# ymLuo1214/RAFT-Stereo

Measured on AMD Instinct MI355X. Metric: stereo pairs/s at 540x960, 32 iters, 1-8 GPUs; corr-lookup HBM GB/s, higher is better.
Workload: dtype f32; 1 GPU; corr path: CorrBlock1D build + 32 lookups, 540x960 -> 135x240 fmaps, batch 8/GPU, fp32, 4 levels, radius 4; config=sceneflow, global_batch=8, W2=240, levels=4, radius=4, iters=32, parallelism=batch-shard x1, corr_out_layout=nchw, pyramid_layout=rows, coords_field=random

## Files before the change

raft-stereo_amd/csrc/lookup_pair.h:

```cpp
#pragma once
#include <type_traits>

#include "common.h"
#include "lookup_level.h"

namespace rc {

template <class OT>
__device__ __forceinline__ OT out_cvt(float v) {
    if constexpr (std::is_same<OT, float>::value) {
        return v;
    } else {
        asm("" : "+v"(v));
        return (OT)v;
    }
}

template <int S>
__device__ __forceinline__ float pool_tree(const float *v) {
    if constexpr (S == 1) return v[0];
    else return (pool_tree<S / 2>(v) + pool_tree<S / 2>(v + S / 2)) * 0.5f;
}

template <int SI>
__device__ __forceinline__ float derived_elem(const float *row1, long long k) {
    float v[SI];
#pragma unroll
    for (int c = 0; c < SI; ++c) v[c] = row1[SI * k + c];
    return pool_tree<SI>(v);
}

template <int R, bool BF16 = false>
struct PairSpan {
    static constexpr int NW = 2 * R + 4;
    static constexpr int NS = 2 * NW;
    static constexpr int EPC = BF16 ? 8 : 4;
    static constexpr int ES = BF16 ? 2 : 4;
    static constexpr int NC = (NS + EPC - 2 + EPC - 1) / EPC;
    uint32_t q[NC][4];
    float m, n;
    int sh;
    bool inwin, valid;
    __device__ __forceinline__ float elem(int e) const {
        if constexpr (BF16) {
            const uint32_t u = q[e >> 3][(e & 7) >> 1];
            return __builtin_bit_cast(float, (e & 1) ? (u & 0xFFFF0000u) : (u << 16));
        } else {
            return __builtin_bit_cast(float, q[e >> 2][e & 3]);
        }
    }
};

template <int R>
__device__ __forceinline__ void tap_span(float xl, int W, int &f, int &l) {
    const float Wm1 = (float)(W - 1), half = Wm1 / 2.0f;
    const DivRN dv = div_prep(Wm1);
    const float pa = ((div_rn(2.0f * ((float)(-R) + xl), dv) - 1.0f) + 1.0f) * half;
    const float pb = ((div_rn(2.0f * ((float)R + xl), dv) - 1.0f) + 1.0f) * half;
    f = max((int)floorf(pa), 0);
    l = min((int)floorf(pb) + 1, W - 1);
}

template <int R, bool BF16 = false>
__device__ __forceinline__ void issue_pair(PairSpan<R, BF16> &ps, const LookupArgs &a, int lo, float x,
                                           long long pblk, long long lrow) {
    typedef PairSpan<R, BF16> PS;
    const int Wlo = a.W[lo], Whi = a.W[lo + 1];
    const float xlo = x / (float)(1 << lo), xhi = x / (float)(2 << lo);
    ps.inwin = (xhi > -(float)(R + 4)) && (xhi < (float)(Whi + R + 4));
    ps.m = ps.inwin ? floorf(xhi) : 0.0f;
    ps.n = ps.inwin ? floorf(xlo) : 0.0f;
    const int dd = (int)ps.n - 2 * (int)ps.m;
    ps.valid = ps.inwin && (dd == 0 || dd == 1);
    int lo_e = 0x7FFFFFFF, hi_e = -1;
    if (ps.inwin) {
        int f, l;
        tap_span<R>(xlo, Wlo, f, l);
        if (f <= l) { lo_e = f; hi_e = l; }
        tap_span<R>(xhi, Whi, f, l);
        if (f <= l) { lo_e = min(lo_e, 2 * f); hi_e = max(hi_e, 2 * l + 1); }
    }
    const int sa = 2 * ((int)ps.m - R - 1);
    const int ea = sa & ~(PS::EPC - 1);
    ps.sh = sa - ea;
    const long long ld = a.ld[lo];
    const char *lvl = static_cast<const char *>(a.lvl[lo]);
    const long long shb = a.shadow[lo];
    const auto rs = make_rsrc(lvl + pblk * ld * PS::ES, clamp_bytes((a.P - pblk) * ld * PS::ES + shb));
    uint32_t phase = 0;
    if (shb != 0 && lo_e <= hi_e) {
        const unsigned long long b0 =
            (unsigned long long)(uintptr_t)(lvl + ((pblk + lrow) * ld + (lo_e & ~(PS::EPC - 1))) * PS::ES);
        const unsigned long long b1 = (unsigned long long)(uintptr_t)(lvl + ((pblk + lrow) * ld + hi_e) * PS::ES);
        const unsigned long long sh = (unsigned long long)shb;
        const long long l0 = (long long)(b1 >> 7) - (long long)(b0 >> 7);
        const long long l1 = (long long)((b1 + sh) >> 7) - (long long)((b0 + sh) >> 7);
        phase = l1 < l0 ? (uint32_t)sh : 0u;
    }
#pragma unroll
    for (int k = 0; k < PS::NC; ++k) {
        const int cs = ea + PS::EPC * k;
        const bool ok = cs <= hi_e && cs + PS::EPC - 1 >= lo_e;
        const auto v = __builtin_amdgcn_raw_buffer_load_b128(
            rs, ok ? (int)((uint32_t)((lrow * ld + cs) * PS::ES) + phase) : (int)0xFFFFFF00u, 0, 0);
#pragma unroll
        for (int c = 0; c < 4; ++c) ps.q[k][c] = v[c];
    }
}

template <int R>
__device__ __forceinline__ void window_taps(const float *w, float xl, float nwin, int W,
                                            float *res) {
    constexpr int T = 2 * R + 1;
    const float Wm1 = (float)(W - 1), half = Wm1 / 2.0f;
    const DivRN dv = div_prep(Wm1);
#pragma unroll
    for (int t = 0; t < T; ++t) {
        const float xt = (float)(t - R) + xl;
        const float xn = div_rn(2.0f * xt, dv) - 1.0f;
        const float xp = (xn + 1.0f) * half;
        const float x0 = floorf(xp);
        const float w1 = xp - x0, w0 = 1.0f - w1;
        const float nt = nwin + (float)(t - R);
        const bool lo_ = x0 < nt, hi_ = x0 > nt;
        float e0 = w[t], e1 = w[t + 1], e2 = w[t + 2], e3 = w[t + 3];
        asm("" : "+v"(e0), "+v"(e1), "+v"(e2), "+v"(e3));
        const float v0 = lo_ ? e0 : (hi_ ? e2 : e1);
        const float v1 = lo_ ? e1 : (hi_ ? e3 : e2);
        res[t] = fmaf(w1, v1, w0 * v0);
    }
}

template <int S>
__device__ __forceinline__ float derived_elem_bf16(const uint16_t *row, long long k) {
    if constexpr (S == 1) {
        return bf16_to_f32(row[k]);
    } else {
        const float a = derived_elem_bf16<S / 2>(row, 2 * k), b = derived_elem_bf16<S / 2>(row, 2 * k + 1);
        return round_bf16((a + b) * 0.5f);
    }
}

template <int R, int S, bool BF16 = false>
__device__ __forceinline__ void level_taps_mem(const void *rowv, float xl, int W, float *res) {
    constexpr int T = 2 * R + 1;
    const float Wm1 = (float)(W - 1), half = Wm1 / 2.0f;
    const DivRN dv = div_prep(Wm1);
    for (int t = 0; t < T; ++t) {
        const float xt = (float)(t - R) + xl;
        const float xn = div_rn(2.0f * xt, dv) - 1.0f;
        const float xp = (xn + 1.0f) * half;
        const float x0 = floorf(xp);
        const float w1 = xp - x0, w0 = 1.0f - w1;
        const bool ok0 = (x0 >= 0.0f) && (x0 <= Wm1);
        const bool ok1 = (x0 + 1.0f >= 0.0f) && (x0 + 1.0f <= Wm1);
        float v0 = 0.0f, v1 = 0.0f;
        if constexpr (BF16) {
            const uint16_t *row = static_cast<const uint16_t *>(rowv);
            if (ok0) v0 = derived_elem_bf16<S>(row, (long long)x0);
            if (ok1) v1 = derived_elem_bf16<S>(row, (long long)x0 + 1);
        } else {
            const float *row = static_cast<const float *>(rowv);
            if (ok0) v0 = derived_elem<S>(row, (long long)x0);
            if (ok1) v1 = derived_elem<S>(row, (long long)x0 + 1);
        }
        res[t] = fmaf(w1, v1, w0 * v0);
    }
}

template <int R, bool NOFALLBACK = false, bool BF16 = false, class Sink>
__device__ __forceinline__ void finish_pair(const PairSpan<R, BF16> &ps, const LookupArgs &a, int lo,
                                            float x, long long pp, Sink &&sink) {
    typedef PairSpan<R, BF16> PS;
    constexpr int T = 2 * R + 1, NW = PS::NW, NS = PS::NS, EPC = PS::EPC;
    const int Wlo = a.W[lo], Whi = a.W[lo + 1];
    float s[NS];
#pragma unroll
    for (int j = 0; j < NS; ++j) {
        float v = ps.elem(j);
#pragma unroll
        for (int d = 2; d < EPC; d += 2)
            if (j + d < PS::NC * EPC) v = (ps.sh == d) ? ps.elem(j + d) : v;
        s[j] = v;
    }
    const int mi = (int)ps.m - R - 1, ni = (int)ps.n - R - 1;
    const int dd = (int)ps.n - 2 * (int)ps.m;
    float wodd[NW], weven[NW];
#pragma unroll
    for (int jj = 0; jj < NW; ++jj) {
        float pm = (s[2 * jj] + s[2 * jj + 1]) * 0.5f;
        if constexpr (BF16) pm = round_bf16(pm);
        wodd[jj] = (unsigned)(mi + jj) < (unsigned)Whi ? pm : 0.0f;
        const float e = dd == 0 ? s[R + 1 + jj] : s[R + 2 + jj];
        weven[jj] = (unsigned)(ni + jj) < (unsigned)Wlo ? e : 0.0f;
    }
    const float xlo = x / (float)(1 << lo), xhi = x / (float)(2 << lo);
    float r0[T], r1[T];
    window_taps<R>(weven, xlo, ps.n, Wlo, r0);
    window_taps<R>(wodd, xhi, ps.m, Whi, r1);
    if (!NOFALLBACK && __builtin_expect(ps.inwin && !ps.valid, 0)) {
        const char *row = static_cast<const char *>(a.lvl[lo]) + pp * a.ld[lo] * PS::ES;
        level_taps_mem<R, 1, BF16>(row, xlo, Wlo, r0);
        level_taps_mem<R, 2, BF16>(row, xhi, Whi, r1);
    }
#pragma unroll
    for (int t = 0; t < T; ++t) sink(lo * T + t, r0[t]);
#pragma unroll
    for (int t = 0; t < T; ++t) sink((lo + 1) * T + t, r1[t]);
}

struct PairPixel {
    long long pblk, pp, lrow;
    long long ooff;
    float x;
    bool active;
};

template <int R, int NL>
__device__ __forceinline__ PairPixel pair_pixel(const LookupArgs &a, long long pblk) {
    PairPixel q;
    q.pblk = pblk;
    const long long p = pblk + threadIdx.x;
    q.active = p < a.P;
    q.pp = q.active ? p : a.P - 1;
    const long long bimg = q.pp / a.HW, rem = q.pp - bimg * a.HW;
    q.x = pixel_x(a, bimg, rem, q.active);
    q.ooff = bimg * (long long)(NL * (2 * R + 1)) * a.HW + rem;
    q.lrow = q.pp - pblk;
    return q;
}

template <int R, int NL, int M = 0, bool BF16 = false, int WPE = 1, bool CL = false, class OT = float>
__global__ __launch_bounds__(256) __attribute__((amdgpu_waves_per_eu(WPE))) void lookup_pair_kernel(LookupArgs a) {
    static_assert(NL == 2 || NL == 4, "pair lookup: 2 or 4 levels");
    constexpr int NP = NL / 2;
    const int blk = M == 5 ? (int)blockIdx.x : xcd_remap(blockIdx.x, gridDim.x);
    const PairPixel q = pair_pixel<R, NL>(a, (long long)blk * 256);
    OT *const outp = reinterpret_cast<OT *>(a.out) + q.ooff;
    PairSpan<R, BF16> sp[NP];
#pragma unroll
    for (int k = 0; k < NP; ++k)
        issue_pair<R, BF16>(sp[k], a, 2 * k, q.x, q.pblk, q.lrow);
    constexpr int C = NL * (2 * R + 1);
    constexpr bool TILE = CL || M == 9;
    __shared__ __attribute__((aligned(16))) OT ctile[TILE ? 4 * 64 * C : 1];
    auto sink = [&](int ch, float v) {
        if constexpr (TILE) {
            ctile[(threadIdx.x >> 6) * 64 * C + (threadIdx.x & 63) * C + ch] = out_cvt<OT>(v);
        } else if constexpr (M == 7) {
            if (q.active) __builtin_nontemporal_store(v, outp + (long long)ch * a.HW);
        } else {
            if (q.active && (M != 1 || v == 1234.5f)) outp[(long long)ch * a.HW] = out_cvt<OT>(v);
        }
    };
#pragma unroll
    for (int k = 0; k < NP; ++k) finish_pair<R, M == 2, BF16>(sp[k], a, 2 * k, q.x, q.pp, sink);
    if constexpr (TILE) {
        constexpr int EPV = 16 / (int)sizeof(OT);
        typedef OT ovec __attribute__((ext_vector_type(EPV)));
        const int lane = threadIdx.x & 63;
        const long long pw = q.pblk + (threadIdx.x & ~63);
        const OT *t = ctile + (threadIdx.x >> 6) * 64 * C;
        OT *const outb = reinterpret_cast<OT *>(a.out);
        const long long lim = (a.P - pw < 64 ? a.P - pw : 64) * C;
#pragma unroll
        for (int k = 0; k < (64 * C / EPV + 63) / 64; ++k) {
            const int e = (k * 64 + lane) * EPV;
            if (e >= 64 * C || e >= lim) continue;
            const ovec v = *reinterpret_cast<const ovec *>(t + e);
            if (e + EPV <= lim) {
                *reinterpret_cast<ovec *>(outb + pw * C + e) = v;
            } else {
#pragma unroll
                for (int j = 0; j < EPV; ++j)
                    if (e + j < lim) outb[pw * C + e + j] = v[j];
            }
        }
    }
}

template <int R, class Sink>
__device__ __forceinline__ void sheared_taps_mem(const LookupArgs &a, int lo, float x, long long bh, int w1,
                                                 Sink &&sink) {
    constexpr int T = 2 * R + 1;
    const float *S = static_cast<const float *>(a.lvl[lo]) + bh * a.shk[lo] * a.ld[lo];
    const int W0 = a.W[lo];
    const long long base = (long long)((w1 >> lo) + W0 - 1);
    auto elem = [&](long long j) { return S[(base - j) * a.ld[lo] + w1]; };
#pragma unroll
    for (int half = 0; half < 2; ++half) {
        const int W = a.W[lo + half];
        const float Wm1 = (float)(W - 1), hw = Wm1 / 2.0f;
        const DivRN dv = div_prep(Wm1);
        const float xl = x / (float)(1 << (lo + half));
        for (int t = 0; t < T; ++t) {
            const float xt = (float)(t - R) + xl;
            const float xn = div_rn(2.0f * xt, dv) - 1.0f;
            const float xp = (xn + 1.0f) * hw;
            const float x0 = floorf(xp);
            const float wt1 = xp - x0, wt0 = 1.0f - wt1;
            const bool ok0 = (x0 >= 0.0f) && (x0 <= Wm1);
            const bool ok1 = (x0 + 1.0f >= 0.0f) && (x0 + 1.0f <= Wm1);
            const long long e = (long long)x0;
            float v0 = 0.0f, v1 = 0.0f;
            if (half == 0) {
                if (ok0) v0 = elem(e);
                if (ok1) v1 = elem(e + 1);
            } else {
                if (ok0) v0 = (elem(2 * e) + elem(2 * e + 1)) * 0.5f;
                if (ok1) v1 = (elem(2 * e + 2) + elem(2 * e + 3)) * 0.5f;
            }
            sink((lo + half) * T + t, fmaf(wt1, v1, wt0 * v0));
        }
    }
}

template <int R, int NL>
__global__ __launch_bounds__(256) void lookup_sheared_pair_kernel(LookupArgs a) {
    static_assert(NL == 2 || NL == 4, "pair lookup: 2 or 4 levels");
    constexpr int NP = NL / 2, NS = PairSpan<R>::NS;
    const int blk = xcd_remap(blockIdx.x, gridDim.x);
    const long long pblk = (long long)blk * 256;
    const long long p = pblk + threadIdx.x;
    const bool active = p < a.P;
    const long long pp = active ? p : a.P - 1;
    const long long bimg = pp / a.HW, rem = pp - bimg * a.HW;
    const float x = pixel_x(a, bimg, rem, active);
    const int H = a.HW / a.W1;
    const int h = (int)(rem / a.W1), w1 = (int)(rem - (long long)h * a.W1);
    const long long bh = bimg * H + h, bh0 = pblk / a.W1;
    float *outp = a.out + bimg * (long long)(NL * (2 * R + 1)) * a.HW + rem;
    auto sink = [&](int ch, float v) {
        if (active) outp[(long long)ch * a.HW] = v;
    };
    PairSpan<R> sp[NP];
#pragma unroll
    for (int k = 0; k < NP; ++k) {
        const int lo = 2 * k;
        PairSpan<R> &ps = sp[k];
        const int Wlo = a.W[lo], Whi = a.W[lo + 1];
        const float xlo = x / (float)(1 << lo), xhi = x / (float)(2 << lo);
        ps.inwin = (xhi > -(float)(R + 4)) && (xhi < (float)(Whi + R + 4));
        ps.m = ps.inwin ? floorf(xhi) : 0.0f;
        ps.n = ps.inwin ? floorf(xlo) : 0.0f;
        const int dd = (int)ps.n - 2 * (int)ps.m;
        ps.valid = ps.inwin && (dd == 0 || dd == 1);
        int lo_e = 0x7FFFFFFF, hi_e = -1;
        if (ps.inwin) {
            int f, l;
            tap_span<R>(xlo, Wlo, f, l);
            if (f <= l) { lo_e = f; hi_e = l; }
            tap_span<R>(xhi, Whi, f, l);
            if (f <= l) { lo_e = min(lo_e, 2 * f); hi_e = max(hi_e, 2 * l + 1); }
        }
        ps.sh = 0;
        const int sa = 2 * ((int)ps.m - R - 1);
        const long long K = a.shk[lo], ldw = a.ld[lo];
        const float *lv = static_cast<const float *>(a.lvl[lo]);
        const auto rs = make_rsrc(lv + bh0 * K * ldw, clamp_bytes((a.P / a.W1 - bh0) * K * ldw * 4));
        const long long rowk = (bh - bh0) * K + (w1 >> lo) + Wlo - 1;
#pragma unroll
        for (int c = 0; c < PairSpan<R>::NC * 4; ++c) {
            const int j = sa + c;
            const bool ok = c < NS && j >= lo_e && j <= hi_e;
            const uint32_t off = ok ? (uint32_t)(((rowk - j) * ldw + w1) * 4) : 0xFFFFFF00u;
            ps.q[c >> 2][c & 3] = __builtin_amdgcn_raw_buffer_load_b32(rs, (int)off, 0, 0);
        }
    }
#pragma unroll
    for (int k = 0; k < NP; ++k) {
        if (__builtin_expect(sp[k].inwin && !sp[k].valid, 0)) {
            sheared_taps_mem<R>(a, 2 * k, x, bh, w1, sink);
            continue;
        }
        finish_pair<R, true>(sp[k], a, 2 * k, x, pp, sink);
    }
}


template <int R>
__device__ __forceinline__ int plan_record_pair(PairSpan<R, true> &ps, const LookupArgs &a, int lo, float x,
                                                int e_first, int slot_first, uint32_t &okmask) {
    typedef PairSpan<R, true> PS;
    const int Wlo = a.W[lo], Whi = a.W[lo + 1];
    const float xlo = x / (float)(1 << lo), xhi = x / (float)(2 << lo);
    ps.inwin = (xhi > -(float)(R + 4)) && (xhi < (float)(Whi + R + 4));
    ps.m = ps.inwin ? floorf(xhi) : 0.0f;
    ps.n = ps.inwin ? floorf(xlo) : 0.0f;
    const int dd = (int)ps.n - 2 * (int)ps.m;
    ps.valid = ps.inwin && (dd == 0 || dd == 1);
    int lo_e = 0x7FFFFFFF, hi_e = -1;
    if (ps.inwin) {
        int f, l;
        tap_span<R>(xlo, Wlo, f, l);
        if (f <= l) { lo_e = f; hi_e = l; }
        tap_span<R>(xhi, Whi, f, l);
        if (f <= l) { lo_e = min(lo_e, 2 * f); hi_e = max(hi_e, 2 * l + 1); }
    }
    const int sslot = 2 * ((int)ps.m - R - 1) - e_first + slot_first;
    const int cb = sslot >= 0 ? sslot & ~7 : -((-sslot + 7) & ~7);
    ps.sh = sslot - cb;
    const int slo = lo_e - e_first + slot_first, shi = hi_e - e_first + slot_first;
    okmask = 0;
#pragma unroll
    for (int k = 0; k < PS::NC; ++k) {
        const int cs = cb + 8 * k;
        if (lo_e <= hi_e && cs <= shi && cs + 7 >= slo && cs >= 0 && cs + 8 <= kRecSlots) okmask |= 1u << k;
    }
    return cb;
}

template <int R, bool NOLOAD = false>
__device__ __forceinline__ void issue_record_pair(PairSpan<R, true> &ps, const LookupArgs &a, int lo, float x,
                                                  const __amdgpu_buffer_rsrc_t &rs, uint32_t rbyte, int e_first,
                                                  int slot_first) {
    typedef PairSpan<R, true> PS;
    uint32_t okm;
    const int cb = plan_record_pair<R>(ps, a, lo, x, e_first, slot_first, okm);
#pragma unroll
    for (int k = 0; k < PS::NC; ++k) {
        const int cs = cb + 8 * k;
        const bool ok = (okm >> k) & 1u;
        if constexpr (NOLOAD) {
            uint32_t o = ok ? rbyte + 2u * (uint32_t)cs : 0u;
            asm volatile("" : "+v"(o));
#pragma unroll
            for (int c = 0; c < 4; ++c) ps.q[k][c] = o + c;
        } else {
            const auto v = __builtin_amdgcn_raw_buffer_load_b128(
                rs, ok ? (int)(rbyte + 2u * (uint32_t)cs) : (int)0xFFFFFF00u, 0, 0);
#pragma unroll
            for (int c = 0; c < 4; ++c) ps.q[k][c] = v[c];
        }
    }
}

template <int R>
__device__ __forceinline__ void lds_record_pair(PairSpan<R, true> &ps, const LookupArgs &a, int lo, float x,
                                                const char *rec, int e_first, int slot_first) {
    typedef PairSpan<R, true> PS;
    uint32_t okm;
    const int cb = plan_record_pair<R>(ps, a, lo, x, e_first, slot_first, okm);
#pragma unroll
    for (int k = 0; k < PS::NC; ++k) {
        const int cs = cb + 8 * k;
        uint4 v = uint4{0u, 0u, 0u, 0u};
        if ((okm >> k) & 1u) v = *reinterpret_cast<const uint4 *>(rec + 2 * cs);
        ps.q[k][0] = v.x;
        ps.q[k][1] = v.y;
        ps.q[k][2] = v.z;
        ps.q[k][3] = v.w;
    }
}

template <int R, class Sink>
__device__ __forceinline__ void record_taps_mem(const LookupArgs &a, const uint16_t *rec, int lo, float x,
                                                Sink &&sink) {
    constexpr int T = 2 * R + 1;
    const int NR = a.rec_nr;
    auto elem = [&](long long e) {
        int r = lo == 0 ? (int)((e - rec_e0(0)) >> 4) : (int)((e - rec_e2(0)) >> 2);
        r = r < NR ? r : NR - 1;
        const int slot = lo == 0 ? kRecL2Slots + (int)e - rec_e0(r) : (int)e - rec_e2(r);
        return bf16_to_f32(rec[r * kRecSlots + slot]);
    };
#pragma unroll
    for (int half = 0; half < 2; ++half) {
        const int W = a.W[lo + half];
        const float Wm1 = (float)(W - 1), hw = Wm1 / 2.0f;
        const DivRN dv = div_prep(Wm1);
        const float xl = x / (float)(1 << (lo + half));
        for (int t = 0; t < T; ++t) {
            const float xt = (float)(t - R) + xl;
            const float xn = div_rn(2.0f * xt, dv) - 1.0f;
            const float xp = (xn + 1.0f) * hw;
            const float x0 = floorf(xp);
            const float wt1 = xp - x0, wt0 = 1.0f - wt1;
            const bool ok0 = (x0 >= 0.0f) && (x0 <= Wm1);
            const bool ok1 = (x0 + 1.0f >= 0.0f) && (x0 + 1.0f <= Wm1);
            const long long e = (long long)x0;
            float v0 = 0.0f, v1 = 0.0f;
            if (half == 0) {
                if (ok0) v0 = elem(e);
                if (ok1) v1 = elem(e + 1);
            } else {
                if (ok0) v0 = round_bf16((elem(2 * e) + elem(2 * e + 1)) * 0.5f);
                if (ok1) v1 = round_bf16((elem(2 * e + 2) + elem(2 * e + 3)) * 0.5f);
            }
            sink((lo + half) * T + t, fmaf(wt1, v1, wt0 * v0));
        }
    }
}

template <int R, bool CL, int M = 0, bool COOP = false, int WPE = 1, class OT = float>
__global__ __launch_bounds__(256) __attribute__((amdgpu_waves_per_eu(WPE))) void lookup_records_kernel(LookupArgs a) {
    constexpr int NL = 4, C = NL * (2 * R + 1);
    const int blk = xcd_remap(blockIdx.x, gridDim.x);
    const PairPixel q = pair_pixel<R, NL>(a, (long long)blk * 256);
    const int NR = a.rec_nr;
    float mf = floorf(q.x / 2.0f);
    mf = fminf(fmaxf(mf, (float)kRecM0), (float)(kRecM0 + 8 * NR - 1));
    const int r = ((int)mf - kRecM0) >> 3;
    const uint16_t *blkrec = static_cast<const uint16_t *>(a.lvl[0]) + q.pblk * (long long)NR * kRecSlots;
    const auto rs = make_rsrc(blkrec, clamp_bytes((a.P - q.pblk) * (long long)NR * kRecSlots * 2));
    const uint32_t rbyte = (uint32_t)((q.lrow * NR + r) * kRecSlots * 2);
    PairSpan<R, true> sp[2];
    constexpr int TB = 64 * C * (int)sizeof(OT);
    constexpr int WB = CL ? (COOP && TB < 8192 ? 8192 : TB) : (COOP ? 8192 : 16);
    __shared__ __attribute__((aligned(16))) char lds[4 * WB];
    char *wlds = lds + (threadIdx.x >> 6) * WB;
    if constexpr (COOP) {
        typedef __attribute__((address_space(3))) void lds_void;
        const int lane = threadIdx.x & 63;
#pragma unroll
        for (int k = 0; k < 8; ++k) {
            const uint32_t rb = (uint32_t)__shfl((int)rbyte, 8 * k + (lane >> 3), 64);
            const int wp = (int)(threadIdx.x & ~63) + 8 * k + (lane >> 3);
            const uint32_t off = q.pblk + wp < a.P ? rb + 16u * (uint32_t)(lane & 7) : 0xFFFFFF00u;
            __builtin_amdgcn_raw_ptr_buffer_load_lds(rs, (lds_void *)(wlds + 1024 * k), 16, (int)off, 0, 0, 0);
        }
        asm volatile("s_waitcnt vmcnt(0)" ::: "memory");
        const char *myrec = wlds + 128 * lane;
        lds_record_pair<R>(sp[0], a, 0, q.x, myrec, rec_e0(r), kRecL2Slots);
        lds_record_pair<R>(sp[1], a, 2, q.x, myrec, rec_e2(r), 0);
        asm volatile("s_waitcnt lgkmcnt(0)" ::: "memory");
    } else {
        issue_record_pair<R, M == 2>(sp[0], a, 0, q.x, rs, rbyte, rec_e0(r), kRecL2Slots);
        issue_record_pair<R, M == 2>(sp[1], a, 2, q.x, rs, rbyte, rec_e2(r), 0);
    }
    if constexpr (M == 3) {
        uint32_t acc = 0;
#pragma unroll
        for (int k = 0; k < 2; ++k)
#pragma unroll
            for (int j = 0; j < PairSpan<R, true>::NC; ++j) acc ^= sp[k].q[j][0] ^ sp[k].q[j][1] ^ sp[k].q[j][2] ^ sp[k].q[j][3];
        asm volatile("" ::"v"(acc));
        return;
    }
    OT *const ctw = reinterpret_cast<OT *>(wlds);
    OT *const outp = reinterpret_cast<OT *>(a.out) + q.ooff;
    auto sink = [&](int ch, float v) {
        if constexpr (CL) ctw[(threadIdx.x & 63) * C + ch] = out_cvt<OT>(v);
        else if (q.active) outp[(long long)ch * a.HW] = out_cvt<OT>(v);
    };
#pragma unroll
    for (int k = 0; k < 2; ++k) {
        if (__builtin_expect(sp[k].inwin && !sp[k].valid, 0)) {
            record_taps_mem<R>(a, blkrec + q.lrow * (long long)NR * kRecSlots, 2 * k, q.x, sink);
            continue;
        }
        finish_pair<R, true, true>(sp[k], a, 2 * k, q.x, q.pp, sink);
    }
    if constexpr (CL) {
        const int lane = threadIdx.x & 63;
        const long long pw = q.pblk + (threadIdx.x & ~63);
        constexpr int EPV = 16 / (int)sizeof(OT);
        typedef OT ovec __attribute__((ext_vector_type(EPV)));
        const OT *t = ctw;
        OT *const outb = reinterpret_cast<OT *>(a.out);
        const long long lim = (a.P - pw < 64 ? a.P - pw : 64) * C;
#pragma unroll
        for (int k = 0; k < (64 * C / EPV + 63) / 64; ++k) {
            const int e = (k * 64 + lane) * EPV;
            if (e >= 64 * C || e >= lim) continue;
            const ovec v = *reinterpret_cast<const ovec *>(t + e);
            if constexpr (M == 1) {
                asm volatile("" ::"v"(v));
            } else if (e + EPV <= lim) {
                *reinterpret_cast<ovec *>(outb + pw * C + e) = v;
            } else {
#pragma unroll
                for (int j = 0; j < EPV; ++j)
                    if (e + j < lim) outb[pw * C + e + j] = v[j];
            }
        }
    }
}

}
```

Baseline: 8405 pairs/s.

## Stagger second level-pair loads behind first pair's tap compute and reuse endpoint taps

The pair kernel now plans and issues the buffer loads for the first level pair, then defers the second pair's loads until after the first pair's even-level taps have been emitted. Scheduling barriers pin this order so the second pair's memory latency can overlap compute while fewer registers are live at once. Tap-span endpoint positions are computed once in a shared planning helper and reused for the first and last taps in window_taps, which removes duplicated divisions. The changes add scheduling constraints that could serialise work if the compiler's own ordering was already better.

```diff
diff --git a/raft-stereo_amd/csrc/lookup_pair.h b/raft-stereo_amd/csrc/lookup_pair.h
--- a/raft-stereo_amd/csrc/lookup_pair.h
+++ b/raft-stereo_amd/csrc/lookup_pair.h
@@ -39,6 +39,7 @@
     static constexpr int NC = (NS + EPC - 2 + EPC - 1) / EPC;
     uint32_t q[NC][4];
     float m, n;
+    float xe[4];
     int sh;
     bool inwin, valid;
     __device__ __forceinline__ float elem(int e) const {
@@ -51,20 +52,24 @@
     }
 };
 
-template <int R>
-__device__ __forceinline__ void tap_span(float xl, int W, int &f, int &l) {
-    const float Wm1 = (float)(W - 1), half = Wm1 / 2.0f;
-    const DivRN dv = div_prep(Wm1);
-    const float pa = ((div_rn(2.0f * ((float)(-R) + xl), dv) - 1.0f) + 1.0f) * half;
-    const float pb = ((div_rn(2.0f * ((float)R + xl), dv) - 1.0f) + 1.0f) * half;
-    f = max((int)floorf(pa), 0);
-    l = min((int)floorf(pb) + 1, W - 1);
-}
-
-template <int R, bool BF16 = false>
-__device__ __forceinline__ void issue_pair(PairSpan<R, BF16> &ps, const LookupArgs &a, int lo, float x,
-                                           long long pblk, long long lrow) {
-    typedef PairSpan<R, BF16> PS;
+struct LevelConsts {
+    float Wm1, half;
+    DivRN dv;
+};
+__device__ __forceinline__ LevelConsts level_consts(const LookupArgs &a, int i) {
+    const float Wm1 = (float)(a.W[i] - 1);
+    return LevelConsts{Wm1, Wm1 / 2.0f, div_prep(Wm1)};
+}
+
+__device__ __forceinline__ float tap_xp(float xl, int k, const LevelConsts &c) {
+    const float xt = (float)k + xl;
+    const float xn = div_rn(2.0f * xt, c.dv) - 1.0f;
+    return (xn + 1.0f) * c.half;
+}
+
+template <int R, bool BF16>
+__device__ __forceinline__ void plan_pair(PairSpan<R, BF16> &ps, const LookupArgs &a, int lo, float x,
+                                          int &lo_e, int &hi_e) {
     const int Wlo = a.W[lo], Whi = a.W[lo + 1];
     const float xlo = x / (float)(1 << lo), xhi = x / (float)(2 << lo);
     ps.inwin = (xhi > -(float)(R + 4)) && (xhi < (float)(Whi + R + 4));
@@ -72,21 +77,42 @@
     ps.n = ps.inwin ? floorf(xlo) : 0.0f;
     const int dd = (int)ps.n - 2 * (int)ps.m;
     ps.valid = ps.inwin && (dd == 0 || dd == 1);
-    int lo_e = 0x7FFFFFFF, hi_e = -1;
+    const LevelConsts clo = level_consts(a, lo), chi = level_consts(a, lo + 1);
+    ps.xe[0] = tap_xp(xlo, -R, clo);
+    ps.xe[1] = tap_xp(xlo, R, clo);
+    ps.xe[2] = tap_xp(xhi, -R, chi);
+    ps.xe[3] = tap_xp(xhi, R, chi);
+    lo_e = 0x7FFFFFFF;
+    hi_e = -1;
     if (ps.inwin) {
-        int f, l;
-        tap_span<R>(xlo, Wlo, f, l);
+        int f = max((int)floorf(ps.xe[0]), 0), l = min((int)floorf(ps.xe[1]) + 1, Wlo - 1);
         if (f <= l) { lo_e = f; hi_e = l; }
-        tap_span<R>(xhi, Whi, f, l);
+        f = max((int)floorf(ps.xe[2]), 0);
+        l = min((int)floorf(ps.xe[3]) + 1, Whi - 1);
         if (f <= l) { lo_e = min(lo_e, 2 * f); hi_e = max(hi_e, 2 * l + 1); }
     }
+}
+
+template <int R, bool BF16>
+struct PairLoads {
+    __amdgpu_buffer_rsrc_t rs;
+    int off[PairSpan<R, BF16>::NC];
+};
+
+template <int R, bool BF16 = false>
+__device__ __forceinline__ PairLoads<R, BF16> plan_pair_loads(PairSpan<R, BF16> &ps, const LookupArgs &a, int lo,
+                                                              float x, long long pblk, long long lrow) {
+    typedef PairSpan<R, BF16> PS;
+    int lo_e, hi_e;
+    plan_pair<R, BF16>(ps, a, lo, x, lo_e, hi_e);
     const int sa = 2 * ((int)ps.m - R - 1);
     const int ea = sa & ~(PS::EPC - 1);
     ps.sh = sa - ea;
     const long long ld = a.ld[lo];
     const char *lvl = static_cast<const char *>(a.lvl[lo]);
     const long long shb = a.shadow[lo];
-    const auto rs = make_rsrc(lvl + pblk * ld * PS::ES, clamp_bytes((a.P - pblk) * ld * PS::ES + shb));
+    PairLoads<R, BF16> pl;
+    pl.rs = make_rsrc(lvl + pblk * ld * PS::ES, clamp_bytes((a.P - pblk) * ld * PS::ES + shb));
     uint32_t phase = 0;
     if (shb != 0 && lo_e <= hi_e) {
         const unsigned long long b0 =
@@ -101,32 +127,40 @@
     for (int k = 0; k < PS::NC; ++k) {
         const int cs = ea + PS::EPC * k;
         const bool ok = cs <= hi_e && cs + PS::EPC - 1 >= lo_e;
-        const auto v = __builtin_amdgcn_raw_buffer_load_b128(
-            rs, ok ? (int)((uint32_t)((lrow * ld + cs) * PS::ES) + phase) : (int)0xFFFFFF00u, 0, 0);
+        pl.off[k] = ok ? (int)((uint32_t)((lrow * ld + cs) * PS::ES) + phase) : (int)0xFFFFFF00u;
+    }
+    return pl;
+}
+
+template <int R, bool BF16>
+__device__ __forceinline__ void load_pair(PairSpan<R, BF16> &ps, const PairLoads<R, BF16> &pl) {
+#pragma unroll
+    for (int k = 0; k < PairSpan<R, BF16>::NC; ++k) {
+        const auto v = __builtin_amdgcn_raw_buffer_load_b128(pl.rs, pl.off[k], 0, 0);
 #pragma unroll
         for (int c = 0; c < 4; ++c) ps.q[k][c] = v[c];
     }
 }
 
 template <int R>
-__device__ __forceinline__ void window_taps(const float *w, float xl, float nwin, int W,
-                                            float *res) {
-    constexpr int T = 2 * R + 1;
-    const float Wm1 = (float)(W - 1), half = Wm1 / 2.0f;
-    const DivRN dv = div_prep(Wm1);
+__device__ __forceinline__ void window_taps(const float *w, float xl, float nwin, const LevelConsts &lc,
+                                            float xa, float xb, float *res) {
+    constexpr int T = 2 * R + 1, NW = 2 * R + 4;
+    float e[NW];
+#pragma unroll
+    for (int j = 0; j < NW; ++j) {
+        e[j] = w[j];
+        asm("" : "+v"(e[j]));
+    }
 #pragma unroll
     for (int t = 0; t < T; ++t) {
-        const float xt = (float)(t - R) + xl;
-        const float xn = div_rn(2.0f * xt, dv) - 1.0f;
-        const float xp = (xn + 1.0f) * half;
+        const float xp = t == 0 ? xa : (t == T - 1 ? xb : tap_xp(xl, t - R, lc));
         const float x0 = floorf(xp);
         const float w1 = xp - x0, w0 = 1.0f - w1;
         const float nt = nwin + (float)(t - R);
         const bool lo_ = x0 < nt, hi_ = x0 > nt;
-        float e0 = w[t], e1 = w[t + 1], e2 = w[t + 2], e3 = w[t + 3];
-        asm("" : "+v"(e0), "+v"(e1), "+v"(e2), "+v"(e3));
-        const float v0 = lo_ ? e0 : (hi_ ? e2 : e1);
-        const float v1 = lo_ ? e1 : (hi_ ? e3 : e2);
+        const float v0 = lo_ ? e[t] : (hi_ ? e[t + 2] : e[t + 1]);
+        const float v1 = lo_ ? e[t + 1] : (hi_ ? e[t + 3] : e[t + 2]);
         res[t] = fmaf(w1, v1, w0 * v0);
     }
 }
@@ -142,14 +176,11 @@
 }
 
 template <int R, int S, bool BF16 = false>
-__device__ __forceinline__ void level_taps_mem(const void *rowv, float xl, int W, float *res) {
+__device__ __forceinline__ void level_taps_mem(const void *rowv, float xl, const LevelConsts &lc, float *res) {
     constexpr int T = 2 * R + 1;
-    const float Wm1 = (float)(W - 1), half = Wm1 / 2.0f;
-    const DivRN dv = div_prep(Wm1);
+    const float Wm1 = lc.Wm1;
     for (int t = 0; t < T; ++t) {
-        const float xt = (float)(t - R) + xl;
-        const float xn = div_rn(2.0f * xt, dv) - 1.0f;
-        const float xp = (xn + 1.0f) * half;
+        const float xp = tap_xp(xl, t - R, lc);
         const float x0 = floorf(xp);
         const float w1 = xp - x0, w0 = 1.0f - w1;
         const bool ok0 = (x0 >= 0.0f) && (x0 <= Wm1);
@@ -168,24 +199,31 @@
     }
 }
 
-template <int R, bool NOFALLBACK = false, bool BF16 = false, class Sink>
-__device__ __forceinline__ void finish_pair(const PairSpan<R, BF16> &ps, const LookupArgs &a, int lo,
-                                            float x, long long pp, Sink &&sink) {
+template <int R, bool BF16>
+__device__ __forceinline__ void span_shift(const PairSpan<R, BF16> &ps, float *s) {
     typedef PairSpan<R, BF16> PS;
-    constexpr int T = 2 * R + 1, NW = PS::NW, NS = PS::NS, EPC = PS::EPC;
+#pragma unroll
+    for (int j = 0; j < PS::NS; ++j) {
+        float v = ps.elem(j);
+#pragma unroll
+        for (int d = 2; d < PS::EPC; d += 2)
+            if (j + d < PS::NC * PS::EPC) v = (ps.sh == d) ? ps.elem(j + d) : v;
+        s[j] = v;
+    }
+}
+
+template <int R, bool NOFALLBACK = false, bool BF16 = false, class Sink, class Mid>
+__device__ __forceinline__ void finish_span(const PairSpan<R, BF16> &ps, const float *s, const LookupArgs &a,
+                                            int lo, float x, long long pp, Sink &&sink, Mid &&mid) {
+    typedef PairSpan<R, BF16> PS;
+    constexpr int T = 2 * R + 1, NW = PS::NW;
     const int Wlo = a.W[lo], Whi = a.W[lo + 1];
-    float s[NS];
-#pragma unroll
-    for (int j = 0; j < NS; ++j) {
-        float v = ps.elem(j);
-#pragma unroll
-        for (int d = 2; d < EPC; d += 2)
-            if (j + d < PS::NC * EPC) v = (ps.sh == d) ? ps.elem(j + d) : v;
-        s[j] = v;
-    }
     const int mi = (int)ps.m - R - 1, ni = (int)ps.n - R - 1;
     const int dd = (int)ps.n - 2 * (int)ps.m;
-    float wodd[NW], weven[NW];
+    const float xlo = x / (float)(1 << lo), xhi = x / (float)(2 << lo);
+    const bool mem = !NOFALLBACK && ps.inwin && !ps.valid;
+    const char *row = static_cast<const char *>(a.lvl[lo]) + pp * a.ld[lo] * PS::ES;
+    float weven[NW], wodd[NW];
 #pragma unroll
     for (int jj = 0; jj < NW; ++jj) {
         float pm = (s[2 * jj] + s[2 * jj + 1]) * 0.5f;
@@ -194,19 +232,25 @@
         const float e = dd == 0 ? s[R + 1 + jj] : s[R + 2 + jj];
         weven[jj] = (unsigned)(ni + jj) < (unsigned)Wlo ? e : 0.0f;
     }
-    const float xlo = x / (float)(1 << lo), xhi = x / (float)(2 << lo);
-    float r0[T], r1[T];
-    window_taps<R>(weven, xlo, ps.n, Wlo, r0);
-    window_taps<R>(wodd, xhi, ps.m, Whi, r1);
-    if (!NOFALLBACK && __builtin_expect(ps.inwin && !ps.valid, 0)) {
-        const char *row = static_cast<const char *>(a.lvl[lo]) + pp * a.ld[lo] * PS::ES;
-        level_taps_mem<R, 1, BF16>(row, xlo, Wlo, r0);
-        level_taps_mem<R, 2, BF16>(row, xhi, Whi, r1);
-    }
-#pragma unroll
-    for (int t = 0; t < T; ++t) sink(lo * T + t, r0[t]);
-#pragma unroll
-    for (int t = 0; t < T; ++t) sink((lo + 1) * T + t, r1[t]);
+    const LevelConsts clo = level_consts(a, lo), chi = level_consts(a, lo + 1);
+    float r[T];
+    window_taps<R>(weven, xlo, ps.n, clo, ps.xe[0], ps.xe[1], r);
+    if (__builtin_expect(mem, 0)) level_taps_mem<R, 1, BF16>(row, xlo, clo, r);
+#pragma unroll
+    for (int t = 0; t < T; ++t) sink(lo * T + t, r[t]);
+    mid();
+    window_taps<R>(wodd, xhi, ps.m, chi, ps.xe[2], ps.xe[3], r);
+    if (__builtin_expect(mem, 0)) level_taps_mem<R, 2, BF16>(row, xhi, chi, r);
+#pragma unroll
+    for (int t = 0; t < T; ++t) sink((lo + 1) * T + t, r[t]);
+}
+
+template <int R, bool NOFALLBACK = false, bool BF16 = false, class Sink>
+__device__ __forceinline__ void finish_pair(const PairSpan<R, BF16> &ps, const LookupArgs &a, int lo,
+                                            float x, long long pp, Sink &&sink) {
+    float s[PairSpan<R, BF16>::NS];
+    span_shift<R, BF16>(ps, s);
+    finish_span<R, NOFALLBACK, BF16>(ps, s, a, lo, x, pp, sink, [] {});
 }
 
 struct PairPixel {
@@ -238,9 +282,11 @@
     const PairPixel q = pair_pixel<R, NL>(a, (long long)blk * 256);
     OT *const outp = reinterpret_cast<OT *>(a.out) + q.ooff;
     PairSpan<R, BF16> sp[NP];
-#pragma unroll
-    for (int k = 0; k < NP; ++k)
-        issue_pair<R, BF16>(sp[k], a, 2 * k, q.x, q.pblk, q.lrow);
+    PairLoads<R, BF16> pl[NP];
+    pl[0] = plan_pair_loads<R, BF16>(sp[0], a, 0, q.x, q.pblk, q.lrow);
+    load_pair<R, BF16>(sp[0], pl[0]);
+    __builtin_amdgcn_sched_barrier(0);
+    if constexpr (NP > 1) pl[1] = plan_pair_loads<R, BF16>(sp[1], a, 2, q.x, q.pblk, q.lrow);
     constexpr int C = NL * (2 * R + 1);
     constexpr bool TILE = CL || M == 9;
     __shared__ __attribute__((aligned(16))) OT ctile[TILE ? 4 * 64 * C : 1];
@@ -254,7 +300,21 @@
         }
     };
 #pragma unroll
-    for (int k = 0; k < NP; ++k) finish_pair<R, M == 2, BF16>(sp[k], a, 2 * k, q.x, q.pp, sink);
+    for (int k = 0; k < NP; ++k) {
+        float s[PairSpan<R, BF16>::NS];
+        span_shift<R, BF16>(sp[k], s);
+        auto next = [&] {
+            if constexpr (NP > 1) {
+                if (k == 0) {
+                    __builtin_amdgcn_sched_barrier(0);
+                    load_pair<R, BF16>(sp[1], pl[1]);
+                    __builtin_amdgcn_sched_barrier(0);
+                }
+            }
+        };
+        finish_span<R, M == 2, BF16>(sp[k], s, a, 2 * k, q.x, q.pp, sink, next);
+        __builtin_amdgcn_sched_barrier(0);
+    }
     if constexpr (TILE) {
         constexpr int EPV = 16 / (int)sizeof(OT);
         typedef OT ovec __attribute__((ext_vector_type(EPV)));
@@ -289,14 +349,11 @@
     auto elem = [&](long long j) { return S[(base - j) * a.ld[lo] + w1]; };
 #pragma unroll
     for (int half = 0; half < 2; ++half) {
-        const int W = a.W[lo + half];
-        const float Wm1 = (float)(W - 1), hw = Wm1 / 2.0f;
-        const DivRN dv = div_prep(Wm1);
+        const LevelConsts lc = level_consts(a, lo + half);
+        const float Wm1 = lc.Wm1;
         const float xl = x / (float)(1 << (lo + half));
         for (int t = 0; t < T; ++t) {
-            const float xt = (float)(t - R) + xl;
-            const float xn = div_rn(2.0f * xt, dv) - 1.0f;
-            const float xp = (xn + 1.0f) * hw;
+            const float xp = tap_xp(xl, t - R, lc);
             const float x0 = floorf(xp);
             const float wt1 = xp - x0, wt0 = 1.0f - wt1;
             const bool ok0 = (x0 >= 0.0f) && (x0 <= Wm1);
@@ -338,21 +395,9 @@
     for (int k = 0; k < NP; ++k) {
         const int lo = 2 * k;
         PairSpan<R> &ps = sp[k];
-        const int Wlo = a.W[lo], Whi = a.W[lo + 1];
-        const float xlo = x / (float)(1 << lo), xhi = x / (float)(2 << lo);
-        ps.inwin = (xhi > -(float)(R + 4)) && (xhi < (float)(Whi + R + 4));
-        ps.m = ps.inwin ? floorf(xhi) : 0.0f;
-        ps.n = ps.inwin ? floorf(xlo) : 0.0f;
-        const int dd = (int)ps.n - 2 * (int)ps.m;
-        ps.valid = ps.inwin && (dd == 0 || dd == 1);
-        int lo_e = 0x7FFFFFFF, hi_e = -1;
-        if (ps.inwin) {
-            int f, l;
-            tap_span<R>(xlo, Wlo, f, l);
-            if (f <= l) { lo_e = f; hi_e = l; }
-            tap_span<R>(xhi, Whi, f, l);
-            if (f <= l) { lo_e = min(lo_e, 2 * f); hi_e = max(hi_e, 2 * l + 1); }
-        }
+        const int Wlo = a.W[lo];
+        int lo_e, hi_e;
+        plan_pair<R, false>(ps, a, lo, x, lo_e, hi_e);
         ps.sh = 0;
         const int sa = 2 * ((int)ps.m - R - 1);
         const long long K = a.shk[lo], ldw = a.ld[lo];
@@ -382,21 +427,8 @@
 __device__ __forceinline__ int plan_record_pair(PairSpan<R, true> &ps, const LookupArgs &a, int lo, float x,
                                                 int e_first, int slot_first, uint32_t &okmask) {
     typedef PairSpan<R, true> PS;
-    const int Wlo = a.W[lo], Whi = a.W[lo + 1];
-    const float xlo = x / (float)(1 << lo), xhi = x / (float)(2 << lo);
-    ps.inwin = (xhi > -(float)(R + 4)) && (xhi < (float)(Whi + R + 4));
-    ps.m = ps.inwin ? floorf(xhi) : 0.0f;
-    ps.n = ps.inwin ? floorf(xlo) : 0.0f;
-    const int dd = (int)ps.n - 2 * (int)ps.m;
-    ps.valid = ps.inwin && (dd == 0 || dd == 1);
-    int lo_e = 0x7FFFFFFF, hi_e = -1;
-    if (ps.inwin) {
-        int f, l;
-        tap_span<R>(xlo, Wlo, f, l);
-        if (f <= l) { lo_e = f; hi_e = l; }
-        tap_span<R>(xhi, Whi, f, l);
-        if (f <= l) { lo_e = min(lo_e, 2 * f); hi_e = max(hi_e, 2 * l + 1); }
-    }
+    int lo_e, hi_e;
+    plan_pair<R, true>(ps, a, lo, x, lo_e, hi_e);
     const int sslot = 2 * ((int)ps.m - R - 1) - e_first + slot_first;
     const int cb = sslot >= 0 ? sslot & ~7 : -((-sslot + 7) & ~7);
     ps.sh = sslot - cb;
@@ -466,14 +498,11 @@
     };
 #pragma unroll
     for (int half = 0; half < 2; ++half) {
-        const int W = a.W[lo + half];
-        const float Wm1 = (float)(W - 1), hw = Wm1 / 2.0f;
-        const DivRN dv = div_prep(Wm1);
+        const LevelConsts lc = level_consts(a, lo + half);
+        const float Wm1 = lc.Wm1;
         const float xl = x / (float)(1 << (lo + half));
         for (int t = 0; t < T; ++t) {
-            const float xt = (float)(t - R) + xl;
-            const float xn = div_rn(2.0f * xt, dv) - 1.0f;
-            const float xp = (xn + 1.0f) * hw;
+            const float xp = tap_xp(xl, t - R, lc);
             const float x0 = floorf(xp);
             const float wt1 = xp - x0, wt0 = 1.0f - wt1;
             const bool ok0 = (x0 >= 0.0f) && (x0 <= Wm1);
```

New measurement: 8745 pairs/s (median of 6 runs). +4.0%, better.
